# noisystreet/aither

Hardware: AMD Instinct MI355X
Metric: Mcell-updates/sec per iteration (residual+LU-SGS), 256^3 block; % HBM roofline (higher is better)
Workload: dtype f64

## Files before the change

### aither_amd/csrc/agx_api.hip

```cpp
#include "agx_kernels.hpp"
#include "agx_geometry.hpp"
#include "agx_mem.hpp"
#include <rccl/rccl.h>
#include <cstdarg>
#include <cstdio>
#include <cstring>
#include <cstdlib>
#include <cmath>
#include <vector>
#include <array>
#include <map>
#include <string>
#include <algorithm>

using namespace agx;

static char g_err[512] = "";
static int fail(const char* fmt, ...) {
  va_list ap;
  va_start(ap, fmt);
  vsnprintf(g_err, sizeof g_err, fmt, ap);
  va_end(ap);
  return 1;
}
// ... 1466 lines not shown
  if (cfg->equation_set != AGX_EQN_RANS || !cfg->is_viscous)
    return fail("the 7-equation library serves equation_set rans (viscous) only");
  if (cfg->turbulence_model != AGX_TURB_SST2003 && cfg->turbulence_model != AGX_TURB_KW_WILCOX2006 &&
      cfg->turbulence_model != AGX_TURB_SST_DES)
    return fail("turbulence_model %d: sst2003, sstdes and kOmegaWilcox2006 are built",
                cfg->turbulence_model);
  if (cfg->inv_flux_jacobian == AGX_JACOBIAN_APPROX_ROE)
    return fail("rans: approximateRoe is not built");
#else
  if (cfg->equation_set != AGX_EQN_EULER && cfg->equation_set != AGX_EQN_NAVIER_STOKES)
    return fail("equation_set %d: this library covers euler and navierStokes "
                "(rans: libaither_gfx950_rans.so)", cfg->equation_set);
  if ((cfg->equation_set == AGX_EQN_NAVIER_STOKES) != (cfg->is_viscous != 0))
    return fail("equation_set %d contradicts is_viscous %d", cfg->equation_set, cfg->is_viscous);
  if (cfg->turbulence_model != AGX_TURB_NONE)
    return fail("turbulence_model %d is not built (laminar / inviscid only)",
                cfg->turbulence_model);
#endif
  if (cfg->inv_flux_jacobian != AGX_JACOBIAN_RUSANOV &&
      cfg->inv_flux_jacobian != AGX_JACOBIAN_APPROX_ROE)
    return fail("inv_flux_jacobian %d is not one of rusanov / approximateRoe",
                cfg->inv_flux_jacobian);
  if (cfg->inv_flux_jacobian == AGX_JACOBIAN_APPROX_ROE && cfg->is_viscous)
    return fail("approximateRoe with viscous terms is not built: the reference hands dist and "
                "f1 to RoeOffDiagonal in swapped order (fluxJacobian.cpp:232 vs :240) and "
                "divides by f1 = 0 in laminar runs");
  if (cfg->viscous_recon != AGX_VISC_RECON_CENTRAL &&
      cfg->viscous_recon != AGX_VISC_RECON_CENTRAL_4TH)
    return fail("viscous_recon %d is not one of central / centralFourth", cfg->viscous_recon);
  if (cfg->viscous_recon == AGX_VISC_RECON_CENTRAL_4TH && cfg->n_ghost < 2)
    return fail("centralFourth needs two ghost layers (input::NumberGhostLayers, "
                "input.cpp:1127-1143)");
  if (cfg->matrix_solver < AGX_SOLVER_LUSGS || cfg->matrix_solver > AGX_SOLVER_BDPLUR)
    return fail("matrix_solver %d is not one of lusgs / dplur / blusgs / bdplur",
                cfg->matrix_solver);
  if ((cfg->matrix_solver == AGX_SOLVER_BLUSGS || cfg->matrix_solver == AGX_SOLVER_BDPLUR) &&
      cfg->inv_flux_jacobian == AGX_JACOBIAN_APPROX_ROE)
    return fail("block-matrix solvers are built for inviscidFluxJacobian rusanov only");
  c->cfg = *cfg;
  derive_gas(*cfg, c->gas);
  c->gas.wilcox = cfg->turbulence_model == AGX_TURB_KW_WILCOX2006 ? 1 : 0;
  c->gas.sstdes = cfg->turbulence_model == AGX_TURB_SST_DES ? 1 : 0;
  c->gas.turb_prandtl = c->gas.wilcox ? 8.0 / 9.0 : 0.9;
#if AGX_TPG
  c->gas.err = c->err_dev.get();
#endif
  SolverDev& sp = c->sp;
  sp.diag_add = 0;
  sp.kappa = cfg->kappa;
  sp.theta = cfg->theta;
  sp.zeta = cfg->zeta;
  sp.relax = cfg->matrix_relaxation;
  sp.dual_time_cfl = cfg->dual_time_cfl;
  sp.dt_fixed = cfg->dt_nondim;
  sp.visc_cfl_coeff = cfg->viscous_cfl_coeff;
  sp.viscous = cfg->is_viscous;
  sp.implicit = cfg->time_integration >= AGX_TIME_IMPLICIT_EULER;
  sp.bdf2 = cfg->time_integration == AGX_TIME_BDF2;
  sp.requires_init = cfg->matrix_solver == AGX_SOLVER_DPLUR ||
                     cfg->matrix_solver == AGX_SOLVER_BDPLUR || cfg->matrix_sweeps > 1;
  sp.block = (cfg->matrix_solver == AGX_SOLVER_BLUSGS || cfg->matrix_solver == AGX_SOLVER_BDPLUR) ? 1 : 0;
  sp.time_integration = cfg->time_integration;
  sp.roe_jacobian = cfg->inv_flux_jacobian == AGX_JACOBIAN_APPROX_ROE;
  c->have_cfg = true;
  return 0;
}

int agx_block_create(agx_ctx* c, const agx_block_geom* g, int* block_id) {
  if (!c->have_cfg) return fail("agx_config_set must precede agx_block_create");
  if (g->ng != c->cfg.n_ghost) return fail("block ghost layers != config n_ghost");
  if (g->ni < 1 || g->nj < 1 || g->nk < 1) return fail("empty block");
  const bool from_nodes = g->nodes != nullptr;
  if (from_nodes) {
    const double* arr[9] = {g->farea_i, g->farea_j, g->farea_k, g->vol, g->center, g->width_i,
                            g->width_j, g->width_k, g->wall_dist};
    const char* nm[9] = {"farea_i", "farea_j", "farea_k", "vol", "center", "width_i", "width_j",
                         "width_k", "wall_dist"};
    for (int q = 0; q < 9; ++q)
      if (arr[q])
        return fail("agx_block_create: nodes given together with %s (a block is built from "
                    "its nodes or from the nine arrays)", nm[q]);
  }
  if (!c->blocks.empty() && c->blocks[0].node_built != from_nodes)
    return fail("agx_block_create: a context holds node-built or array-built blocks, not both");
  HIPCHK(hipSetDevice(c->device));
  c->blocks.emplace_back();
  Block& b = c->blocks.back();
  BlockDev& d = b.d;
  memset(&d, 0, sizeof d);
  d.ni = g->ni; d.nj = g->nj; d.nk = g->nk; d.ng = g->ng;
  d.parent = g->parent_block;
  b.global_pos = g->global_pos;
  d.ioff = 16;
  const long row = d.ioff + d.ni + d.ng + 1;
  d.sx = (row + 15) / 16 * 16;
  d.sxy = d.sx * (d.nj + 2 * d.ng + 1);
  d.nplane = d.sxy * (d.nk + 2 * d.ng + 1);
  HIPCHK(b.slab.alloc((size_t)d.nplane * PL_COUNT));
  HIPCHK(hipMemsetAsync(b.slab.get(), 0, sizeof(double) * d.nplane * PL_COUNT, c->stream));
  auto pl = [&](int id) { return b.slab.get() + (long)id * d.nplane; };
  d.vol = pl(PL_VOL); d.specrad = pl(PL_SPECRAD); d.dt = pl(PL_DT);
  d.a = pl(PL_A); d.ainv = pl(PL_AINV); d.wdist = pl(PL_WDIST);
  for (int e = 0; e < AGX_NEQ; ++e) {
    d.state[e] = pl(PL_STATE_A + e); d.state2[e] = pl(PL_STATE_B + e);
    d.resid[e] = pl(PL_RESID + e); d.consn[e] = pl(PL_CONSN + e);
    d.consnm1[e] = pl(PL_CONSNM1 + e); d.x[e] = pl(PL_X + e);
    d.xold[e] = pl(PL_XOLD + e);
  }
  for (int q = 0; q < 3; ++q) {
    d.cen[q] = pl(PL_CEN + q);
    d.wid[q] = pl(PL_WID + q);
    for (int cc = 0; cc < 4; ++cc) d.fa[q][cc] = pl(PL_FA + 4 * q + cc);
  }
  b.state_is_a = true;
#if AGX_NEQ == 7
  d.specrad_t = pl(PL_SPECRAD_T); d.a_t = pl(PL_A_T); d.ainv_t = pl(PL_AINV_T);
  d.viscp = pl(PL_VISC);
  for (int q = 0; q < 3; ++q) d.turb3[q] = pl(PL_TURB3 + q);
#endif
  if (c->sp.implicit && is_block_solver(c)) {
    const size_t n = (size_t)d.nplane * (2 * AGX_NJ + 9 + 4);
    HIPCHK(b.blockmat.alloc(n));
    HIPCHK(hipMemsetAsync(b.blockmat.get(), 0, sizeof(double) * n, c->stream));
    d.am = b.blockmat.get();
    d.aminv = d.am + (size_t)d.nplane * AGX_NJ;
    d.vg = d.am + (size_t)d.nplane * 2 * AGX_NJ;
    d.am_t = d.vg + (size_t)d.nplane * 9;
    d.aminv_t = d.am_t + (size_t)d.nplane * 2;
  }
  d.sw_geo = d.sw_dyn = d.sw_rhs = nullptr;
  d.mg_forcing = d.mg_mres = d.mg_xsave = nullptr;
  if (c->sp.implicit && is_lusgs_solver(c) && !use_d2(c) && c->sweep_records) {
    const size_t n = (size_t)d.nplane * (SW_GEO + SW_DYN + SW_RHS);
    HIPCHK(b.sweep_rec.alloc(n));
    HIPCHK(hipMemsetAsync(b.sweep_rec.get(), 0, sizeof(double) * n, c->stream));
    d.sw_geo = b.sweep_rec.get();
    d.sw_dyn = d.sw_geo + (size_t)d.nplane * SW_GEO;
    d.sw_rhs = d.sw_dyn + (size_t)d.nplane * SW_DYN;
  }
  if (use_d2(c) && std::min(d.ni, d.nj) > KP_MAX_DIAG)
    return fail("LU-SGS: a block with min(ni, nj) = %d exceeds the %d cells per diagonal "
                "the sweep kernel holds in LDS (AGX_LUSGS=plane has no such limit)",
                std::min(d.ni, d.nj), KP_MAX_DIAG);
  if (use_d2(c)) {
    D2Dev& z = d.d2;
    z.Pi = d.ni + 2 * d.ng; z.Pj = d.nj + 2 * d.ng;
    z.ps = ((long)z.Pi * z.Pj + 15) / 16 * 16;
    z.nd2 = z.ps * (d.nk + 2 * d.ng);
    b.dstart.assign(z.Pi + z.Pj + 1, 0);
    std::vector<int> tab(z.Pi + z.Pj + 1 + (size_t)z.Pi * z.Pj);
    for (int de = 0; de < z.Pi + z.Pj - 1; ++de) {
      const int jl = std::max(0, de - (z.Pi - 1)), jh = std::min(z.Pj - 1, de);
      b.dstart[de + 1] = b.dstart[de] + (jh - jl + 1);
      for (int je = jl; je <= jh; ++je)
        tab[z.Pi + z.Pj + 1 + b.dstart[de] + (je - jl)] = (de - je) | (je << 16);
    }
    b.dstart[z.Pi + z.Pj] = b.dstart[z.Pi + z.Pj - 1];
    std::copy(b.dstart.begin(), b.dstart.end(), tab.begin());
    HIPCHK(b.d2_tab.upload(tab));
    z.dstart = b.d2_tab.get();
    z.ij_of_pos = z.dstart + z.Pi + z.Pj + 1;
    HIPCHK(b.d2.alloc((size_t)z.nd2 * D2_DOUBLES));
    HIPCHK(hipMemsetAsync(b.d2.get(), 0, sizeof(double) * z.nd2 * D2_DOUBLES, c->stream));
    z.base = b.d2.get();
  }
  b.node_built = from_nodes;
  if (from_nodes) {
    if (geo_block_metrics(c, b, g->nodes)) return 1;
    *block_id = (int)c->blocks.size() - 1;
    return 0;
  }
  const int ci = d.ni + 2 * d.ng, cj = d.nj + 2 * d.ng, ck = d.nk + 2 * d.ng;
  if (upload_aos(c, b, g->farea_i, d.fa[0], 4, ci + 1, cj, ck, d.ng)) return 1;
  if (upload_aos(c, b, g->farea_j, d.fa[1], 4, ci, cj + 1, ck, d.ng)) return 1;
  if (upload_aos(c, b, g->farea_k, d.fa[2], 4, ci, cj, ck + 1, d.ng)) return 1;
  double* volp[1] = {d.vol};
  if (upload_aos(c, b, g->vol, volp, 1, ci, cj, ck, d.ng)) return 1;
  if (upload_aos(c, b, g->center, d.cen, 3, ci, cj, ck, d.ng)) return 1;
  const double* wsrc[3] = {g->width_i, g->width_j, g->width_k};
  for (int q = 0; q < 3; ++q) {
    double* wp[1] = {d.wid[q]};
    if (upload_aos(c, b, wsrc[q], wp, 1, ci, cj, ck, d.ng)) return 1;
  }
#if AGX_FAST
  if (d.d2.base) {
    const long n = (long)d.d2.Pi * d.d2.Pj * (d.nk + 2 * d.ng);
    hipLaunchKernelGGL(k_d2_geo, dim3((n + 255) / 256), dim3(256), 0, c->stream, d);
  }
#endif
  HIPCHK(hipGetLastError());
  if (g->wall_dist) {
    double* wp[1] = {d.wdist};
    if (upload_aos(c, b, g->wall_dist, wp, 1, ci, cj, ck, d.ng)) return 1;
  }
  *block_id = (int)c->blocks.size() - 1;
  return 0;
}

int agx_block_set_bcs(agx_ctx* c, int id, int n, const agx_bc_surface* s) {
  if (id < 0 || id >= (int)c->blocks.size()) return fail("bad block id %d", id);
  Block& b = c->blocks[id];
  b.sweep_graph.drop();
  b.surf_host.assign(s, s + n);
  b.d.surf = nullptr;
  b.d.nsurf = 0;
  HIPCHK(b.surf_dev.alloc(n > 0 ? n : 1));
  HIPCHK(hipMemcpy(b.surf_dev.get(), s, sizeof(agx_bc_surface) * n, hipMemcpyHostToDevice));
  b.d.surf = b.surf_dev.get();
  b.d.nsurf = n;
  b.d.nsurf_i = b.d.nsurf_j = b.d.nsurf_k = 0;
  int n_conn[6] = {0, 0, 0, 0, 0, 0}, n_other[6] = {0, 0, 0, 0, 0, 0};
  for (int q = 0; q < n; ++q) {
    const int st = surface_type(s[q]);
    if (st <= 2) b.d.nsurf_i++; else if (st <= 4) b.d.nsurf_j++; else b.d.nsurf_k++;
    const int t = s[q].bc_type;
    if (t < AGX_BC_SLIPWALL || t > AGX_BC_PERIODIC) return fail("unknown bc type %d", t);
    if (t == AGX_BC_INTERBLOCK || t == AGX_BC_PERIODIC) n_conn[st - 1]++; else n_other[st - 1]++;
    if (t == AGX_BC_VISCOUSWALL && s[q].state.is_wall_law) {
      if (AGX_NEQ == 5) return fail("wallTreatment=wallLaw needs the rans library");
    }
  }
  for (int q = 0; q < 6; ++q)
    b.d.side_conn[q] = n_conn[q] == 0 ? 0 : (n_other[q] == 0 ? 1 : 2);
  b.d.nr_off = nullptr; b.d.nr_grad = nullptr; b.d.nr_mach = nullptr;
  b.nr_off_dev.reset();
  b.nr_mem.reset();
  b.nr_max = 0;
  std::vector<int> off(n > 0 ? n : 1, -1);
  long total = 0, nr_max = 0;
  for (int q = 0; q < n; ++q) {
    const int t = s[q].bc_type;
    if (!s[q].state.is_nonreflecting || (t != AGX_BC_INLET && t != AGX_BC_PRESSURE_OUTLET)) continue;
    const int st = surface_type(s[q]);
    const int d3 = (st - 1) / 2, d1 = (d3 + 1) % 3, d2 = (d3 + 2) % 3;
    const int lo[3] = {s[q].imin, s[q].jmin, s[q].kmin}, hi[3] = {s[q].imax, s[q].jmax, s[q].kmax};
    const long cells = (long)(hi[d1] - lo[d1]) * (hi[d2] - lo[d2]);
    off[q] = (int)total;
    total += cells;
    nr_max = std::max(nr_max, cells);
  }
  if (total > 0) {
    HIPCHK(b.nr_off_dev.upload(off.data(), (size_t)n));
    const size_t nd = (size_t)12 * total + 2 * (size_t)n;
    HIPCHK(b.nr_mem.alloc(nd));
    HIPCHK(hipMemset(b.nr_mem.get(), 0, sizeof(double) * nd));
    b.d.nr_off = b.nr_off_dev.get();
    b.d.nr_grad = b.nr_mem.get();
    b.d.nr_mach = b.nr_mem.get() + 12 * total;
    b.nr_max = nr_max;
  }
  b.d.wall_off = nullptr; b.d.wallv = nullptr;
  b.wall_off_dev.reset();
  b.wall_mem.reset();
  std::fill(off.begin(), off.end(), -1);
  total = 0;
  for (int q = 0; q < n; ++q) {
    if (s[q].bc_type != AGX_BC_VISCOUSWALL || !s[q].state.is_wall_law) continue;
    const int st = surface_type(s[q]);
    const int d3 = (st - 1) / 2, d1 = (d3 + 1) % 3, d2 = (d3 + 2) % 3;
    const int lo[3] = {s[q].imin, s[q].jmin, s[q].kmin}, hi[3] = {s[q].imax, s[q].jmax, s[q].kmax};
    off[q] = (int)total;
    total += (long)(hi[d1] - lo[d1]) * (hi[d2] - lo[d2]);
  }
  if (total > 0) {
    HIPCHK(b.wall_off_dev.upload(off.data(), (size_t)n));
    HIPCHK(b.wall_mem.alloc((size_t)total));
    HIPCHK(hipMemset(b.wall_mem.get(), 0, sizeof(WallVars) * (size_t)total));
    b.d.wall_off = b.wall_off_dev.get();
    b.d.wallv = b.wall_mem.get();
    c->have_wall_data = false;
  }
  b.wall_tab_dev.reset();
  b.wall_tab.clear();
  b.wall_faces = 0;
  for (int q = 0; q < n; ++q) {
    if (s[q].bc_type != AGX_BC_VISCOUSWALL) continue;
    WallSurfDev w;
    const int lo[3] = {s[q].imin, s[q].jmin, s[q].kmin}, hi[3] = {s[q].imax, s[q].jmax, s[q].kmax};
    const int nn[3] = {b.d.ni, b.d.nj, b.d.nk};
    w.side = surface_type(s[q]);
    const int d3 = (w.side - 1) / 2;
    for (int d = 0; d < 3; ++d) {
      w.lo[d] = lo[d];
      w.n[d] = d == d3 ? 1 : hi[d] - lo[d];
      if (lo[d] < 0 || hi[d] > nn[d] || w.n[d] < 1 || (d == d3 && lo[d] != 0 && lo[d] != nn[d]))
        return fail("viscousWall surface %d does not lie on a side of block %d", q, id);
    }
    w.off = b.wall_faces;
    b.wall_faces += (long)w.n[0] * w.n[1] * w.n[2];
    b.wall_tab.push_back(w);
  }
  HIPCHK(b.wall_tab_dev.upload(b.wall_tab));
  return 0;
}

int agx_conn_create(agx_ctx* c, const agx_connection* cc, int* conn_id) {
  c->conns.emplace_back();
  c->conns.back().c = *cc;
  *conn_id = (int)c->conns.size() - 1;
  return 0;
}

#ifndef AGX_MRESID_KC
#define AGX_MRESID_KC 32
#endif
constexpr int MRESID_KC = AGX_MRESID_KC;
long mresid_wgs(const agx_ctx* c, const BlockDev& b) {
  const long nchunk = ((long)b.d2.Pi * b.d2.Pj + 255) / 256;
  if (c->mresid_march) return 8L * ((nchunk + 7) / 8) * ((b.nk + MRESID_KC - 1) / MRESID_KC);
  const long bands = 8L * c->mresid_split;
  return bands * ((nchunk + bands - 1) / bands) * b.nk;
}

namespace {
int halo_batch_plan(agx_ctx* c, long* max_halo) {
  int sides = 0;
  long total = 0;
  std::vector<std::vector<unsigned char>> wlev(c->blocks.size()), rlev(c->blocks.size());
  auto flags = [&](std::vector<std::vector<unsigned char>>& v, int blk) -> std::vector<unsigned char>& {
    if (v[blk].empty()) v[blk].assign((size_t)c->blocks[blk].d.nplane, 0);
    return v[blk];
  };
  std::vector<std::pair<int, int>> order;
  int nlev = 0;
  for (size_t n = 0; n < c->conns.size(); ++n) {
    auto& k = c->conns[n];
    const agx_connection& cc = k.c;
    if (!(cc.rank[0] == c->rank && cc.rank[1] == c->rank)) continue;
    int lev = 1;
    for (int sd = 0; sd < 2; ++sd) {
      const auto& wr = flags(wlev, cc.local_block[1 - sd]);
      for (long q : k.side[sd].h_src) lev = std::max(lev, wr[(size_t)q] + 1);
      const auto& ww = flags(wlev, cc.local_block[sd]);
      const auto& rr = flags(rlev, cc.local_block[sd]);
      for (long q : k.side[sd].h_dst)
        lev = std::max(lev, std::max<int>(ww[(size_t)q] + 1, rr[(size_t)q]));
    }
    lev = std::min(lev, 250);
    for (int sd = 0; sd < 2; ++sd) {
      auto& rr = flags(rlev, cc.local_block[1 - sd]);
      for (long q : k.side[sd].h_src) rr[(size_t)q] = std::max<unsigned char>(rr[(size_t)q], lev);
      auto& ww = flags(wlev, cc.local_block[sd]);
      for (long q : k.side[sd].h_dst) ww[(size_t)q] = (unsigned char)lev;
      total += k.side[sd].n;
    }
    order.emplace_back(lev, (int)n);
    nlev = std::max(nlev, lev);
    sides += 2;
  }
  for (auto& k : c->conns)
    for (int sd = 0; sd < 2; ++sd) {
      std::vector<long>().swap(k.side[sd].h_dst);
      std::vector<long>().swap(k.side[sd].h_src);
    }
  c->halo_batch = c->halo_batch && sides >= 4 && nlev < 250 && 2 * nlev < sides;
  if (!c->halo_batch && c->halo_batch_required)
    return fail("AGX_HALO_BATCH=require: %d local connections in %d levels", sides / 2, nlev);
  if (!c->halo_batch) return 0;
  std::stable_sort(order.begin(), order.end(),
                   [](const std::pair<int, int>& x, const std::pair<int, int>& y) { return x.first < y.first; });
  c->halo_conn_order.clear();
  c->halo_levels.assign(nlev, agx_ctx::HaloLevel{0, 0, 0});
  long nmax_all = 0;
  for (auto& o : order) {
    auto& L = c->halo_levels[o.first - 1];
    if (L.sides == 0) L.first = 2 * (int)c->halo_conn_order.size();
    L.sides += 2;
    const auto& k = c->conns[o.second];
    L.nmax = std::max(L.nmax, std::max(k.side[0].n, k.side[1].n));
    nmax_all = std::max(nmax_all, L.nmax);
    c->halo_conn_order.push_back(o.second);
  }
  c->halo_batch_sides = sides;
  c->halo_batch_nmax = nmax_all;
  *max_halo = std::max(*max_halo, (total * AGX_NEQ + 1) / 2);
  HIPCHK(c->halo_tab_host.alloc((size_t)2 * sides));
  return 0;
}
void halo_sides(agx_ctx* c, Conn& k, int what, double* buf0, double* buf1, HaloSide* g,
                HaloSide* p) {
  Block& b0 = c->blocks[k.c.local_block[0]];
  Block& b1 = c->blocks[k.c.local_block[1]];
  const int z = halo_in_d2(b0, what);
  const auto &m0 = k.side[0].map[z], &m1 = k.side[1].map[z];
  g[0] = HaloSide{halo_planes(b1, what), m0.src.get(), k.side[0].n, buf0};
  g[1] = HaloSide{halo_planes(b0, what), m1.src.get(), k.side[1].n, buf1};
  p[0] = HaloSide{halo_planes(b0, what), m0.dst.get(), k.side[0].n, buf0};
  p[1] = HaloSide{halo_planes(b1, what), m1.dst.get(), k.side[1].n, buf1};
}
int halo_batch_tables(agx_ctx* c, int what) {
  const int set = c->halo_set[what];
  if (c->halo_tab_valid[what][set]) return 0;
  const int sides = c->halo_batch_sides;
  auto& tab = c->halo_tab_dev[what][set];
  for (int q = 0; q < 2; ++q)
    if (!tab[q]) HIPCHK(tab[q].alloc((size_t)sides));
  HIPCHK(hipStreamSynchronize(c->stream));
  HaloSide* g = c->halo_tab_host.get();
  HaloSide* p = g + sides;
  double* buf = c->halo_buf.get();
  int n = 0;
  for (int cid : c->halo_conn_order) {
    auto& k = c->conns[cid];
    const long n0 = k.side[0].n, n1 = k.side[1].n;
    halo_sides(c, k, what, buf, buf + n0 * AGX_NEQ, g + n, p + n);
    buf += (n0 + n1) * AGX_NEQ;
    n += 2;
  }
  HIPCHK(hipMemcpyAsync(tab[0].get(), g, sizeof(HaloSide) * sides, hipMemcpyHostToDevice,
                        c->stream));
  HIPCHK(hipMemcpyAsync(tab[1].get(), p, sizeof(HaloSide) * sides, hipMemcpyHostToDevice,
                        c->stream));
  c->halo_tab_valid[what][set] = true;
  return 0;
}
}

namespace {
struct CellIndex {
  const Block* b;
  int space;
  long operator()(int i, int j, int k) const {
    return !b ? 0L : space ? b->d2idx(i, j, k) : b->d.idx(i, j, k);
  }
};
int halo_maps(Conn& k, int s, int space, int ng, CellIndex idx_mine, CellIndex idx_partner,
              bool partner_local, long* max_halo) {
  MapOut m;
  build_side_map(k.c, s, ng, idx_mine, idx_partner, m);
  if (!partner_local) {
    MapOut ms;
    build_side_map(k.c, 1 - s, ng, idx_partner, idx_mine, ms);
    k.n_send = (long)ms.src.size();
    HIPCHK(k.send_src[space].upload(ms.src));
    *max_halo = std::max(*max_halo, (long)ms.src.size() * AGX_NEQ);
  }
  ConnSide& sd = k.side[s];
  sd.n = (long)m.dst.size();
  HIPCHK(sd.map[space].dst.upload(m.dst));
  if (partner_local) HIPCHK(sd.map[space].src.upload(m.src));
  *max_halo = std::max(*max_halo, (long)m.dst.size() * AGX_NEQ);
  if (space == 0) {
    sd.h_dst = std::move(m.dst);
    if (partner_local) sd.h_src = std::move(m.src);
  }
  return 0;
}
}

int agx_setup_finalize(agx_ctx* c) {
  HIPCHK(hipSetDevice(c->device));
  const int ng = c->cfg.n_ghost;
  if (!c->blocks.empty() && c->blocks[0].node_built && geo_complete(c)) return 1;
  long max_parts = 1, max_halo = 1;
  long march_parts = 0;
  for (auto& blk : c->blocks) {
    const dim3 g = cell_grid(blk.d, CELL_BLOCK);
    max_parts = std::max(max_parts, (long)g.x * g.y * g.z);
    march_parts += march_plan(c, blk.d).nparts;
    if (blk.d.d2.base)
      max_parts = std::max(max_parts, mresid_wgs(c, blk.d));
  }
  max_parts = std::max(max_parts, march_parts);
  for (auto& k : c->conns) {
    const agx_connection& cc = k.c;
    const bool l0 = cc.rank[0] == c->rank, l1 = cc.rank[1] == c->rank;
    if (!l0 && !l1) continue;
    for (int s = 0; s < 2; ++s) {
      const bool mine = s == 0 ? l0 : l1, partner_mine = s == 0 ? l1 : l0;
      if (!mine) continue;
      const int lb = cc.local_block[s];
      if (lb < 0 || lb >= (int)c->blocks.size()) return fail("connection refers to unknown block");
      const Block* partner = partner_mine ? &c->blocks[cc.local_block[1 - s]] : nullptr;
      for (int space = 0; space < (use_d2(c) ? 2 : 1); ++space)
        if (halo_maps(k, s, space, ng, CellIndex{&c->blocks[lb], space},
                      CellIndex{partner, space}, partner_mine, &max_halo))
          return 1;
    }
  }
  if (halo_batch_plan(c, &max_halo)) return 1;
  if (ensure_halo_buf(c, 2 * max_halo)) return 1;
  std::vector<std::pair<int, int>> per_peer;
  for (size_t n = 0; n < c->conns.size(); ++n) {
    if (my_side(c, c->conns[n]) < 0) continue;
    agx_ctx::Remote r;
    r.cid = (int)n;
    r.count = (long)agx_halo_count(c, (int)n, AGX_HALO_STATE);
    const bool hb = c->have_ex && c->ex.host_buffers;
    const size_t cap = (size_t)std::max<long>(r.count, 1);
    HIPCHK(r.send.alloc(cap));
    HIPCHK(r.recv.alloc(cap));
    if (hb) {
      HIPCHK(r.hsend.alloc(cap));
      HIPCHK(r.hrecv.alloc(cap));
    }
    const int s = my_side(c, c->conns[n]);
    agx_slab sl;
    sl.peer = c->conns[n].c.rank[1 - s];
    sl.tag = 0;
    bool seen = false;
    for (auto& pp : per_peer)
      if (pp.first == sl.peer) { sl.tag = pp.second++; seen = true; }
    if (!seen) per_peer.emplace_back(sl.peer, 1);
    sl.count = r.count;
    sl.send = hb ? r.hsend.get() : r.send.get();
    sl.recv = hb ? r.hrecv.get() : r.recv.get();
    c->slabs.push_back(sl);
    c->remote.push_back(std::move(r));
  }
  if (c->have_ex) {
    const size_t nrec = 1 + (size_t)c->ex.nranks;
    HIPCHK(c->rec_dev.alloc(nrec));
    HIPCHK(c->rec_host.alloc(nrec));
  }
  c->n_partials = max_parts;
  HIPCHK(c->partials.alloc((size_t)max_parts));
  const size_t nb = std::max<size_t>(c->blocks.size(), 1);
  HIPCHK(c->norm_out.alloc(2 * nb + 64));
  HIPCHK(c->norm_host.alloc(2 * nb));
  c->finalized = true;
  return 0;
}

int agx_state_upload(agx_ctx* c, int id, const double* state) {
  c->ghosts_prefilled = false;
  c->state_is_time_n = false;
  if (flush_consn(c)) return 1;
  if (id < 0 || id >= (int)c->blocks.size()) return fail("bad block id %d", id);
  Block& b = c->blocks[id];
  const BlockDev& d = b.d;
  if (upload_aos(c, b, state, d.state, AGX_NEQ, d.ni + 2 * d.ng,
                 d.nj + 2 * d.ng, d.nk + 2 * d.ng, d.ng))
    return 1;
#if AGX_NEQ == 7
  hipLaunchKernelGGL(k_aux_field, dim3((d.nplane + 255) / 256), dim3(256), 0, c->stream, d,
                     c->gas, 1, d.viscp);
  HIPCHK(hipGetLastError());
#endif
  return 0;
}

static int field_info(Block& b, int field, double* const** p, int* ncomp, int* ghost) {
  BlockDev& d = b.d;
  static thread_local double* one[1];
  switch (field) {
    case AGX_FIELD_STATE: *p = d.state; *ncomp = AGX_NEQ; *ghost = 1; return 0;
    case AGX_FIELD_RESIDUAL: *p = d.resid; *ncomp = AGX_NEQ; *ghost = 0; return 0;
    case AGX_FIELD_CONS_N: *p = d.consn; *ncomp = AGX_NEQ; *ghost = 0; return 0;
    case AGX_FIELD_CONS_NM1: *p = d.consnm1; *ncomp = AGX_NEQ; *ghost = 0; return 0;
    case AGX_FIELD_UPDATE: *p = d.x; *ncomp = AGX_NEQ; *ghost = 1; return 0;
    case AGX_FIELD_DT: one[0] = d.dt; *p = one; *ncomp = 1; *ghost = 0; return 0;
    case AGX_FIELD_SPEC_RADIUS: one[0] = d.specrad; *p = one; *ncomp = 1; *ghost = 0; return 0;
    case AGX_FIELD_DIAGONAL: one[0] = d.a; *p = one; *ncomp = 1; *ghost = 0; return 0;
  }
  return 1;
}
static int geom_field_info(Block& b, int field, double* const** p, int* ncomp, int* face) {
  BlockDev& d = b.d;
  static thread_local double* one[1];
  *face = -1;
  switch (field) {
    case AGX_FIELD_VOLUME: one[0] = d.vol; *p = one; *ncomp = 1; return 0;
    case AGX_FIELD_CENTER: *p = d.cen; *ncomp = 3; return 0;
    case AGX_FIELD_FAREA_I: case AGX_FIELD_FAREA_J: case AGX_FIELD_FAREA_K:
      *face = field - AGX_FIELD_FAREA_I; *p = d.fa[*face]; *ncomp = 4; return 0;
    case AGX_FIELD_WIDTH_I: case AGX_FIELD_WIDTH_J: case AGX_FIELD_WIDTH_K:
      one[0] = d.wid[field - AGX_FIELD_WIDTH_I]; *p = one; *ncomp = 1; return 0;
    case AGX_FIELD_WALL_DIST: one[0] = d.wdist; *p = one; *ncomp = 1; return 0;
  }
  return 1;
}

static int d2_x_copy(agx_ctx* c, Block& b, int to_d2) {
#if AGX_FAST
  b.x_planes_current = true;
  const long n = (long)b.d.d2.Pi * b.d.d2.Pj * (b.d.nk + 2 * b.d.ng);
  hipLaunchKernelGGL(k_d2_x_copy, dim3((n + 255) / 256), dim3(256), 0, c->stream, b.d, to_d2,
                     to_d2 ? (unsigned)(++b.kp_epoch) & 3u : 0u);
  HIPCHK(hipGetLastError());
#endif
  return 0;
}

static int ghosts_for_output(agx_ctx* c) {
  if (!c->ghosts_prefilled) {
    if (agx_phase_bc_faces(c)) return 1;
    if (agx_halo_swap_local(c, AGX_HALO_STATE)) return 1;
    if (agx_phase_bc_edges(c)) return 1;
  }
  if (c->cfg.is_viscous) {
    if (bc_pass(c, true, 2)) return 1;
    if (bc_pass(c, false, 1)) return 1;
  }
  c->ghosts_prefilled = false;
  return 0;
}

int agx_field_download(agx_ctx* c, int id, int field, double* out) {
  if (flush_consn(c)) return 1;
  if (id < 0 || id >= (int)c->blocks.size()) return fail("bad block id %d", id);
  Block& b = c->blocks[id];
  if (field == AGX_FIELD_UPDATE && b.d.d2.base && d2_x_copy(c, b, 0)) return 1;
  if (field >= AGX_FIELD_VEL_GRAD && field <= AGX_FIELD_PRESS_GRAD) {
    const long ncell = (long)b.d.ni * b.d.nj * b.d.nk;
    double* tmp = nullptr;
    if (ghosts_for_output(c)) return 1;
    if (stage_buffer(c, (size_t)3 * NGF * ncell, &tmp)) return 1;
// ... 1053 lines not shown
```

### aither_amd/csrc/agx_lusgs_kernels.hpp

```cpp
#pragma once

namespace agx {

constexpr int TT = 32;
constexpr int TRS = TT + 2;
__device__ __forceinline__ int tile_diag_index(int li, int lj) {
  const int dd = li + lj;
  if (dd < TT) return dd * (dd + 1) / 2 + lj;
  const int r = 2 * TT - 2 - dd;
  return TT * TT - (r + 1) * (r + 2) / 2 + (lj - (dd - (TT - 1)));
}
__device__ __forceinline__ void tile_table(unsigned short* s_tab) {
  const int tid = threadIdx.x;
#pragma unroll
  for (int m = 0; m < 4; ++m) {
    const int li = tid & (TT - 1), lj = (tid >> 5) + 8 * m;
    s_tab[tile_diag_index(li, lj)] = (unsigned short)(li | (lj << 8));
  }
}

__device__ __forceinline__ double kp_tagged(double v, unsigned tag) {
  const unsigned long long u = (unsigned long long)__double_as_longlong(v);
  return __longlong_as_double((long long)((u & ~3ull) | tag));
}
// ... 262 lines not shown
    const int kq = FWD ? k - 1 : k + 1;
    const bool has_pre = kt > 0;
    const bool k_any = has_pre || (CONN && b.side_conn[FWD ? 4 : 5] != 0);
    const long kbase = (long)(k + ng) * z.ps, qbase = (long)(kq + ng) * z.ps;
    auto step_geom = [&](int t, int& d, int& jmin, int& cnt, int& p0, int& pn) {
      d = FWD ? t : nsteps - 1 - t;
      jmin = max(0, d - (b.ni - 1));
      cnt = min(b.nj - 1, d) - jmin + 1;
      const int de = d + 2 * ng;
      p0 = z.dstart_cf(de) + (jmin + ng) - z.jlo(de);
      const int dq = FWD ? de - 1 : de + 1;
      pn = z.dstart_cf(dq) - z.jlo(dq);
    };
    auto fetch = [&](int t, KpCell* cc) {
      int d, jmin, cnt, p0, pn;
      step_geom(t, d, jmin, cnt, p0, pn);
#pragma unroll
      for (int m = 0; m < CH; ++m) {
        KpCell& c = cc[m];
        const int nraw = tid + 256 * m;
        c.act = nraw < cnt;
        const int n = c.act ? nraw : 0;
        c.j = jmin + n;
        c.i = d - c.j;
        c.pos = p0 + n;
        const unsigned vo = (unsigned)c.pos * 16u;
#pragma unroll
        for (int h = 0; h < 3; ++h) {
          c.o[h] = ld16(z.pab((FWD ? PA_B : PA_X) + h) + kbase * 16, vo);
          c.s[h] = ld16(z.pab(PA_S + h) + kbase * 16, vo);
          c.qs[h] = ld16(z.pab(PA_S + h) + qbase * 16, vo);
        }
        c.vf = ld8(z.vfb() + kbase * 8, (unsigned)c.pos * 8u);
        c.qvf = ld8(z.vfb() + qbase * 8, (unsigned)c.pos * 8u);
        const long fb[3] = {FWD ? kbase : kbase + pn, FWD ? kbase : kbase + pn + 1,
                            FWD ? kbase : kbase + z.ps};
        const unsigned fo[3] = {FWD ? vo : (unsigned)(c.j + ng) * 16u,
                                FWD ? vo : (unsigned)(c.j + ng) * 16u, vo};
#pragma unroll
        for (int q = 0; q < 3; ++q) {
          const double2 t0 = ld16(z.pab(PA_F + 2 * q) + fb[q] * 16, fo[q]);
          const double2 t1 = ld16(z.pab(PA_F + 2 * q + 1) + fb[q] * 16, fo[q]);
          c.f[q].n[0] = t0.x; c.f[q].n[1] = t0.y; c.f[q].n[2] = t1.x; c.f[q].a = t1.y;
          c.f[q].ad = ld8(z.adb(q) + fb[q] * 8, fo[q] >> 1);
        }
        const bool in_i = FWD ? c.i > 0 : c.i < b.ni - 1;
        const bool in_j = FWD ? c.j > 0 : c.j < b.nj - 1;
        int use = (in_i ? 1 : 0) | (in_j ? 2 : 0) | (has_pre ? 4 : 0);
        if (CONN) {
          if (FWD) {
            if (!in_i && bc_is_connection(b, c.i, c.j, k, 1)) use |= 1 | 8;
            if (!in_j && bc_is_connection(b, c.i, c.j, k, 3)) use |= 2 | 16;
            if (!has_pre && bc_is_connection(b, c.i, c.j, k, 5)) use |= 4;
          } else {
            if (!in_i && bc_is_connection(b, c.i + 1, c.j, k, 2)) use |= 1 | 8;
            if (!in_j && bc_is_connection(b, c.i, c.j + 1, k, 4)) use |= 2 | 16;
            if (!has_pre && bc_is_connection(b, c.i, c.j, k + 1, 6)) use |= 4;
          }
        }
        c.use = use;
      }
    };
    KpCell cur[CH], nxt[CH];
    double qx[CH][AGX_NEQ];
    auto qx_request = [&]() {
#pragma unroll
      for (int m = 0; m < CH; ++m) {
#pragma unroll
        for (int e = 0; e < AGX_NEQ; ++e) {
          const double* p = reinterpret_cast<const double*>(
              z.pab(PA_X + (e >> 1)) + qbase * 16 + (unsigned)cur[m].pos * 16u) + (e & 1);
          qx[m][e] = __hip_atomic_load(p, __ATOMIC_RELAXED, __HIP_MEMORY_SCOPE_AGENT);
        }
      }
    };
    auto qx_landed = [&]() {
      unsigned bad = 0;
#pragma unroll
      for (int m = 0; m < CH; ++m) {
#pragma unroll
        for (int e = 0; e < AGX_NEQ; ++e)
          bad |= cur[m].act ? ((unsigned)__double_as_longlong(qx[m][e]) ^ kp.tag) : 0u;
      }
      return (bad & 3u) == 0u;
    };
#pragma unroll
    for (int m = 0; m < CH; ++m) {
      cur[m].act = false;
#pragma unroll
      for (int e = 0; e < AGX_NEQ; ++e) qx[m][e] = 0.0;
    }
    int jmin_prev = 0;
    fetch(0, cur);
    __builtin_amdgcn_s_waitcnt(0x0F70);
    for (int t = 0; t < nsteps; ++t) {
      KP_STAMP(0);
      if (k_any) qx_request();
      fetch(min(t + 1, nsteps - 1), nxt);
      KP_STAMP(1);
      {
        int d, jmin, cnt, p0, pn;
      step_geom(t, d, jmin, cnt, p0, pn);
      double* lw = kp_lds + (size_t)(t & 1) * KP_NV * nsl;
      const double* lr = kp_lds + (size_t)((t & 1) ^ 1) * KP_NV * nsl;
      double accs[CH][AGX_NEQ];
#pragma unroll
      for (int m = 0; m < CH; ++m) {
        const KpCell& c = cur[m];
        double* acc = accs[m];
#pragma unroll
        for (int e = 0; e < AGX_NEQ; ++e) acc[e] = 0.0;
#pragma unroll
        for (int q = 0; q < 2; ++q) {
          const int jn = q == 0 ? c.j : (FWD ? c.j - 1 : c.j + 1);
          const double* rp = lr + min(max(jn - jmin_prev + 1, 0), nsl - 1);
          KpRec r;
#pragma unroll
          for (int e = 0; e < AGX_NEQ; ++e) r.dx[e] = rp[e * nsl];
          r.r1 = rp[5 * nsl]; r.v1[0] = rp[6 * nsl]; r.v1[1] = rp[7 * nsl]; r.v1[2] = rp[8 * nsl];
          r.p1 = rp[9 * nsl]; r.h1 = rp[10 * nsl];
          r.r0 = rp[11 * nsl]; r.v0[0] = rp[12 * nsl]; r.v0[1] = rp[13 * nsl]; r.v0[2] = rp[14 * nsl];
          r.p0 = rp[15 * nsl]; r.h0 = rp[16 * nsl]; r.cs = rp[17 * nsl]; r.vf = rp[18 * nsl];
          if (CONN && (c.use & (8 << q))) {
            const long pg = kbase + pn + (c.j + ng) + (q == 0 ? 0 : (FWD ? -1 : 1));
            kp_term_mem(z, g, visc, pg, c.f[q], FWD, acc);
          } else {
            const bool on = (c.use & (1 << q)) != 0;
            kp_term(r, c.f[q].n, on ? c.f[q].a : 0.0, on ? c.f[q].ad : 0.0, true, FWD, acc);
          }
        }
      }
      KP_STAMP(2);
      if (has_pre) {
        int spins = 0;
        while (!__all(qx_landed())) {
          __builtin_amdgcn_s_sleep(KP_SLEEP);
          if (++spins > kp.spin_limit ||
              ((spins & 63) == 0 &&
               __hip_atomic_load(kp.err, __ATOMIC_RELAXED, __HIP_MEMORY_SCOPE_AGENT) != 0)) {
            s_ok = 0;
            __hip_atomic_store(kp.err, 2, __ATOMIC_RELAXED, __HIP_MEMORY_SCOPE_AGENT);
            break;
          }
          qx_request();
          __builtin_amdgcn_s_waitcnt(0x0F70);
        }
      }
      KP_STAMP(3);
      __builtin_amdgcn_s_waitcnt(0x0F70);
#pragma unroll
      for (int m = 0; m < CH; ++m) {
        const KpCell& c = cur[m];
        double* acc = accs[m];
        const long own = kbase + c.pos;
        if (k_any) {
          const double qs5[AGX_NEQ] = {c.qs[0].x, c.qs[0].y, c.qs[1].x, c.qs[1].y, c.qs[2].x};
          KpRec r;
          kp_build_rec(g, qs5, c.qs[2].y, c.qvf, qx[m], r);
          const bool on = CONN ? (c.use & 4) != 0 : true;
          kp_term(r, c.f[2].n, on ? c.f[2].a : 0.0, on ? c.f[2].ad : 0.0, true, FWD, acc);
        }
        const double ainv = c.o[2].y;
        const double ov[AGX_NEQ] = {c.o[0].x, c.o[0].y, c.o[1].x, c.o[1].y, c.o[2].x};
        double xn[AGX_NEQ];
        if (FULL) {
          const int de = d + 2 * ng;
          const int dqo = FWD ? de + 1 : de - 1;
          const long po = kbase + z.dstart_cf(dqo) - z.jlo(dqo) + (c.j + ng);
          KpFace ff;
          if (FWD) {
            if (c.i < b.ni - 1 || bc_is_connection(b, c.i + 1, c.j, k, 2)) {
              kp_load_face(z, 0, po, visc, ff);
              kp_term_mem(z, g, visc, po, ff, false, acc);
            }
            if (c.j < b.nj - 1 || bc_is_connection(b, c.i, c.j + 1, k, 4)) {
              kp_load_face(z, 1, po + 1, visc, ff);
              kp_term_mem(z, g, visc, po + 1, ff, false, acc);
            }
            if (k < b.nk - 1 || bc_is_connection(b, c.i, c.j, k + 1, 6)) {
              kp_load_face(z, 2, own + z.ps, visc, ff);
              kp_term_mem(z, g, visc, own + z.ps, ff, false, acc);
            }
          } else {
            if (c.i > 0 || bc_is_connection(b, c.i, c.j, k, 1)) {
              kp_load_face(z, 0, own, visc, ff);
              kp_term_mem(z, g, visc, po, ff, true, acc);
            }
            if (c.j > 0 || bc_is_connection(b, c.i, c.j, k, 3)) {
              kp_load_face(z, 1, own, visc, ff);
              kp_term_mem(z, g, visc, po - 1, ff, true, acc);
            }
            if (k > 0 || bc_is_connection(b, c.i, c.j, k, 5)) {
              kp_load_face(z, 2, own, visc, ff);
              kp_term_mem(z, g, visc, own - z.ps, ff, true, acc);
            }
          }
          double bv[AGX_NEQ] = {ov[0], ov[1], ov[2], ov[3], ov[4]};
          if (!FWD) {
            const double2 b0 = z.ld_pair(PA_B, own), b1 = z.ld_pair(PA_B + 1, own),
                          b2 = z.ld_pair(PA_B + 2, own);
            bv[0] = b0.x; bv[1] = b0.y; bv[2] = b1.x; bv[3] = b1.y; bv[4] = b2.x;
          }
#pragma unroll
          for (int e = 0; e < AGX_NEQ; ++e) xn[e] = (bv[e] + acc[e]) * ainv;
        } else if (FWD) {
#pragma unroll
          for (int e = 0; e < AGX_NEQ; ++e) xn[e] = (ov[e] + acc[e]) * ainv;
        } else {
#pragma unroll
          for (int e = 0; e < AGX_NEQ; ++e) xn[e] = ov[e] + acc[e] * ainv;
        }
#pragma unroll
        for (int e = 0; e < AGX_NEQ; ++e) xn[e] = kp_tagged(xn[e], kp.tag);
        if (c.act) {
          typedef double v2d __attribute__((ext_vector_type(2)));
          const unsigned po = (unsigned)c.pos * 16u;
          const v2d v0 = {xn[0], xn[1]}, v1 = {xn[2], xn[3]}, v2 = {xn[4], ainv};
          asm volatile("s_nop 4\n\tglobal_store_dwordx4 %0, %1, %2 sc1\n\ts_nop 1"
                       :: "v"(po), "v"(v0), "s"(z.pab(PA_X + 0) + kbase * 16) : "memory");
          asm volatile("s_nop 4\n\tglobal_store_dwordx4 %0, %1, %2 sc1\n\ts_nop 1"
                       :: "v"(po), "v"(v1), "s"(z.pab(PA_X + 1) + kbase * 16) : "memory");
          asm volatile("s_nop 4\n\tglobal_store_dwordx4 %0, %1, %2 sc1\n\ts_nop 1"
                       :: "v"(po), "v"(v2), "s"(z.pab(PA_X + 2) + kbase * 16) : "memory");
        }
        const double s5[AGX_NEQ] = {c.s[0].x, c.s[0].y, c.s[1].x, c.s[1].y, c.s[2].x};
        KpRec r;
        kp_build_rec(g, s5, c.s[2].y, c.vf, xn, r);
        if (c.act) {
        double* wp = lw + (c.j - jmin + 1);
#pragma unroll
        for (int e = 0; e < AGX_NEQ; ++e) wp[e * nsl] = xn[e];
        wp[5 * nsl] = r.r1; wp[6 * nsl] = r.v1[0]; wp[7 * nsl] = r.v1[1]; wp[8 * nsl] = r.v1[2];
        wp[9 * nsl] = r.p1; wp[10 * nsl] = r.h1;
        wp[11 * nsl] = r.r0; wp[12 * nsl] = r.v0[0]; wp[13 * nsl] = r.v0[1]; wp[14 * nsl] = r.v0[2];
        wp[15 * nsl] = r.p0; wp[16 * nsl] = r.h0; wp[17 * nsl] = r.cs; wp[18 * nsl] = r.vf;
        }
      }
      jmin_prev = jmin;
      }
      KP_STAMP(4);
      __syncthreads();
      if (!s_ok) return;
#pragma unroll
      for (int m = 0; m < CH; ++m) cur[m] = nxt[m];
      KP_STAMP(5);
    }
  }
}

__global__ void __launch_bounds__(256)
k_matrix_resid_d2(BlockDev b, GasDev g, SolverDev sp, int nsplit, NormPartial* partials) {
  const D2Dev& z = b.d2;
  const int nchunk = (z.Pi * z.Pj + 255) / 256;
  const int per = (nchunk + 8 * nsplit - 1) / (8 * nsplit);
  const int xcd = blockIdx.x % 8, m = blockIdx.x / 8;
  const int band = (m / (per * b.nk)) * 8 + xcd, rem = m % (per * b.nk);
  const int k = rem / per, chunk = band * per + rem % per;
  const int t = chunk * 256 + threadIdx.x;
  const bool visc = sp.viscous != 0;
  double r[AGX_NEQ] = {0, 0, 0, 0, 0};
  bool active = false;
  if (chunk < nchunk && t < z.Pi * z.Pj) {
    const int ij = z.ij_of_pos[t];
    const int ie = ij & 0xffff, je = ij >> 16;
    const int i = ie - b.ng, j = je - b.ng;
    active = i >= 0 && i < b.ni && j >= 0 && j < b.nj;
    if (active) {
      const long kbase = (long)(k + b.ng) * z.ps;
      const long own = kbase + t;
      const int de = ie + je;
      const long plo = kbase + z.dstart[de - 1] - z.jlo(de - 1) + je;
      const long pup = kbase + z.dstart[de + 1] - z.jlo(de + 1) + je;
      double acc[AGX_NEQ] = {0, 0, 0, 0, 0};
      const long nlo[3] = {plo, plo - 1, own - z.ps}, nup[3] = {pup, pup + 1, own + z.ps};
      const int c3[3] = {i, j, k}, n3[3] = {b.ni, b.nj, b.nk};
      KpFace ff;
#pragma unroll
      for (int d = 0; d < 3; ++d) {
        if (c3[d] > 0 || bc_is_connection(b, i, j, k, 2 * d + 1)) {
          kp_load_face(z, d, own, visc, ff);
          kp_term_mem(z, g, visc, nlo[d], ff, true, acc);
        }
      }
#pragma unroll
      for (int d = 0; d < 3; ++d) {
        if (c3[d] < n3[d] - 1 ||
            bc_is_connection(b, i + (d == 0), j + (d == 1), k + (d == 2), 2 * d + 2)) {
          kp_load_face(z, d, nup[d], visc, ff);
          kp_term_mem(z, g, visc, nup[d], ff, false, acc);
        }
      }
      const double2 x0 = z.pa(PA_X)[own], x1 = z.pa(PA_X + 1)[own], x2 = z.pa(PA_X + 2)[own];
      const double2 b0 = z.pa(PA_B)[own], b1 = z.pa(PA_B + 1)[own], b2 = z.pa(PA_B + 2)[own];
      const double a = 1.0 / b2.y;
      const double xv[AGX_NEQ] = {x0.x, x0.y, x1.x, x1.y, x2.x};
      const double bv[AGX_NEQ] = {b0.x, b0.y, b1.x, b1.y, b2.x};
#pragma unroll
      for (int e = 0; e < AGX_NEQ; ++e) r[e] = -(xv[e] * a - acc[e] - bv[e]);
    }
  }
  norm_block_reduce(r, 0, active, partials + blockIdx.x);
}

#ifndef AGX_MR_WAVES
#define AGX_MR_WAVES 1
#endif
__global__ void __launch_bounds__(256, AGX_MR_WAVES)
k_matrix_resid_d2m(BlockDev b, GasDev g, SolverDev sp, int kc, NormPartial* partials) {
  const D2Dev& z = b.d2;
  const int nchunk = (z.Pi * z.Pj + 255) / 256;
  const int per = (nchunk + 7) / 8;
  const int xcd = blockIdx.x % 8, m = blockIdx.x / 8;
  const int chunk = xcd * per + m % per, kch = m / per;
  const int k0 = kch * kc, k1 = min(k0 + kc, b.nk);
  const int t = chunk * 256 + threadIdx.x;
  const bool visc = sp.viscous != 0;
  double l2[AGX_NEQ] = {0, 0, 0, 0, 0};
  bool active = false;
  int i = 0, j = 0, je = 0, de = 0;
  if (chunk < nchunk && t < z.Pi * z.Pj) {
    const int ij = z.ij_of_pos[t];
    const int ie = ij & 0xffff;
    je = ij >> 16;
    i = ie - b.ng; j = je - b.ng; de = ie + je;
    active = i >= 0 && i < b.ni && j >= 0 && j < b.nj;
  }
  if (active) {
    const long qlo = z.dstart[de - 1] - z.jlo(de - 1) + je;
    const long qup = z.dstart[de + 1] - z.jlo(de + 1) + je;
    struct Col { double s[AGX_NEQ], cs, x[AGX_NEQ], vf; };
    auto ld_col = [&](long p, Col& c) {
      const double2 s0 = z.ld_pair(PA_S, p), s1 = z.ld_pair(PA_S + 1, p), s2 = z.ld_pair(PA_S + 2, p);
      const double2 x0 = z.ld_pair(PA_X, p), x1 = z.ld_pair(PA_X + 1, p), x2 = z.ld_pair(PA_X + 2, p);
      c.s[0] = s0.x; c.s[1] = s0.y; c.s[2] = s1.x; c.s[3] = s1.y; c.s[4] = s2.x; c.cs = s2.y;
      c.x[0] = x0.x; c.x[1] = x0.y; c.x[2] = x1.x; c.x[3] = x1.y; c.x[4] = x2.x;
      c.vf = visc ? z.ld_vf(p) : 0.0;
    };
    auto col_term = [&](const Col& c, const KpFace& f, bool lower, double* acc) {
      KpRec r;
      kp_build_rec(g, c.s, c.cs, c.vf, c.x, r);
      kp_term(r, f.n, f.a, f.ad, visc, lower, acc);
    };
    Col cm, c0, cp;
    KpFace fk0, fk1;
    long own = (long)(k0 + b.ng) * z.ps + t;
    ld_col(own - z.ps, cm);
    ld_col(own, c0);
    kp_load_face(z, 2, own, visc, fk0);
    for (int k = k0; k < k1; ++k, own += z.ps) {
      const long kbase = own - t;
      ld_col(own + z.ps, cp);
      kp_load_face(z, 2, own + z.ps, visc, fk1);
      const double2 b0 = z.pa(PA_B)[own], b1 = z.pa(PA_B + 1)[own], b2 = z.pa(PA_B + 2)[own];
      double acc[AGX_NEQ] = {0, 0, 0, 0, 0};
      KpFace ff;
      if (i > 0 || bc_is_connection(b, i, j, k, 1)) {
        kp_load_face(z, 0, own, visc, ff);
        kp_term_mem(z, g, visc, kbase + qlo, ff, true, acc);
      }
      if (j > 0 || bc_is_connection(b, i, j, k, 3)) {
        kp_load_face(z, 1, own, visc, ff);
        kp_term_mem(z, g, visc, kbase + qlo - 1, ff, true, acc);
      }
      if (k > 0 || bc_is_connection(b, i, j, k, 5)) col_term(cm, fk0, true, acc);
      if (i < b.ni - 1 || bc_is_connection(b, i + 1, j, k, 2)) {
        kp_load_face(z, 0, kbase + qup, visc, ff);
        kp_term_mem(z, g, visc, kbase + qup, ff, false, acc);
      }
      if (j < b.nj - 1 || bc_is_connection(b, i, j + 1, k, 4)) {
        kp_load_face(z, 1, kbase + qup + 1, visc, ff);
        kp_term_mem(z, g, visc, kbase + qup + 1, ff, false, acc);
      }
      if (k < b.nk - 1 || bc_is_connection(b, i, j, k + 1, 6)) col_term(cp, fk1, false, acc);
      const double a = 1.0 / b2.y;
      const double bv[AGX_NEQ] = {b0.x, b0.y, b1.x, b1.y, b2.x};
#pragma unroll
      for (int e = 0; e < AGX_NEQ; ++e) {
        const double r = -(c0.x[e] * a - acc[e] - bv[e]);
        l2[e] += r * r;
      }
      cm = c0; c0 = cp; fk0 = fk1;
    }
  }
  norm_block_fold(l2, -1.0e300, 0x7fffffffffffffffLL, partials + blockIdx.x);
}

__global__ void __launch_bounds__(256)
k_update_d2(BlockDev b, GasDev g, SolverDev sp, int last_mm, NormPartial* partials) {
  __shared__ double sv[AGX_NEQ][TT][TRS];
  __shared__ unsigned short s_tab[TT * TT];
  const D2Dev& z = b.d2;
  const int tid = threadIdx.x;
  tile_table(s_tab);
  __syncthreads();
  const int i0 = blockIdx.x * TT, j0 = blockIdx.y * TT, k = blockIdx.z;
#pragma unroll
  for (int m = 0; m < 4; ++m) {
    const unsigned tl = s_tab[tid + 256 * m];
    const int tli = tl & 0xff, tlj = tl >> 8;
    const int i = i0 + tli, j = j0 + tlj;
    if (i < b.ni && j < b.nj) {
      const long p = (long)(k + b.ng) * z.ps + z.pos2(i + b.ng, j + b.ng);
      const double2 x0 = z.pa(PA_X)[p], x1 = z.pa(PA_X + 1)[p], x2 = z.pa(PA_X + 2)[p];
      sv[0][tlj][tli] = x0.x; sv[1][tlj][tli] = x0.y; sv[2][tlj][tli] = x1.x;
      sv[3][tlj][tli] = x1.y; sv[4][tlj][tli] = x2.x;
    }
  }
  __syncthreads();
  const int li = tid & (TT - 1);
  double l2[AGX_NEQ] = {0, 0, 0, 0, 0};
  double vmax = -1.0e300;
  long long vlin = 0x7fffffffffffffffLL;
#pragma unroll
  for (int m = 0; m < 4; ++m) {
    const int lj = (tid >> 5) + 8 * m;
    const int i = i0 + li, j = j0 + lj;
    if (i < b.ni && j < b.nj) {
      const long q = b.idx(i, j, k);
      double r[AGX_NEQ], s[AGX_NEQ], du[AGX_NEQ], ns[AGX_NEQ];
      load5(b.resid, q, r);
      load5(b.state, q, s);
#pragma unroll
      for (int e = 0; e < AGX_NEQ; ++e) du[e] = sv[e][lj][li];
      update_prim_with_cons(g, s, du, ns);
      store5(b.state, q, ns);
      if (sp.bdf2 && last_mm) {
        double u[AGX_NEQ];
        load5(b.consn, q, u);
        store5(b.consnm1, q, u);
      }
      const long lin0 = (((long)k * b.nj + j) * b.ni + i) * AGX_NEQ;
#pragma unroll
      for (int e = 0; e < AGX_NEQ; ++e) {
        l2[e] += r[e] * r[e];
        if (r[e] > vmax || (r[e] == vmax && lin0 + e < vlin)) { vmax = r[e]; vlin = lin0 + e; }
      }
    }
  }
  const long bid = ((long)blockIdx.z * gridDim.y + blockIdx.y) * gridDim.x + blockIdx.x;
  norm_block_fold(l2, vmax, vlin, partials + bid);
}

}
```

Measured before the change: 1477.

## Share i/j neighbor columns via wave shuffles in matrix residual kernel

Reworks the k-marching matrix-residual kernel so that the i-neighbor column is loaded once per plane and the j-neighbor column is obtained from the adjacent lane via __shfl_up/__shfl_down, falling back to a memory load only when that lane is inactive or out of range. The k-march now keeps two columns instead of three and reuses a single k-face load. The k chunk size is halved to expose more workgroups. These changes aim to cut redundant global loads of neighbor state, at the cost of extra shuffle instructions and possible register pressure, and they assume that adjacent lanes in the diagonal layout really hold the j-neighbors.

```diff
diff --git a/aither_amd/csrc/agx_api.hip b/aither_amd/csrc/agx_api.hip
--- a/aither_amd/csrc/agx_api.hip
+++ b/aither_amd/csrc/agx_api.hip
@@ -1792,7 +1792,7 @@
 }
 
 #ifndef AGX_MRESID_KC
-#define AGX_MRESID_KC 32
+#define AGX_MRESID_KC 16
 #endif
 constexpr int MRESID_KC = AGX_MRESID_KC;
 long mresid_wgs(const agx_ctx* c, const BlockDev& b) {
diff --git a/aither_amd/csrc/agx_lusgs_kernels.hpp b/aither_amd/csrc/agx_lusgs_kernels.hpp
--- a/aither_amd/csrc/agx_lusgs_kernels.hpp
+++ b/aither_amd/csrc/agx_lusgs_kernels.hpp
@@ -588,22 +588,18 @@
   norm_block_reduce(r, 0, active, partials + blockIdx.x);
 }
 
-#ifndef AGX_MR_WAVES
-#define AGX_MR_WAVES 1
-#endif
-__global__ void __launch_bounds__(256, AGX_MR_WAVES)
+__global__ void __launch_bounds__(256, 1)
 k_matrix_resid_d2m(BlockDev b, GasDev g, SolverDev sp, int kc, NormPartial* partials) {
   const D2Dev& z = b.d2;
+  const bool visc = sp.viscous != 0;
+  double l2[AGX_NEQ] = {0, 0, 0, 0, 0};
+  bool active = false;
+  int i = 0, j = 0, je = 0, de = 0, t = 0;
   const int nchunk = (z.Pi * z.Pj + 255) / 256;
   const int per = (nchunk + 7) / 8;
   const int xcd = blockIdx.x % 8, m = blockIdx.x / 8;
   const int chunk = xcd * per + m % per, kch = m / per;
-  const int k0 = kch * kc, k1 = min(k0 + kc, b.nk);
-  const int t = chunk * 256 + threadIdx.x;
-  const bool visc = sp.viscous != 0;
-  double l2[AGX_NEQ] = {0, 0, 0, 0, 0};
-  bool active = false;
-  int i = 0, j = 0, je = 0, de = 0;
+  t = chunk * 256 + threadIdx.x;
   if (chunk < nchunk && t < z.Pi * z.Pj) {
     const int ij = z.ij_of_pos[t];
     const int ie = ij & 0xffff;
@@ -611,6 +607,11 @@
     i = ie - b.ng; j = je - b.ng; de = ie + je;
     active = i >= 0 && i < b.ni && j >= 0 && j < b.nj;
   }
+  const int k0 = kch * kc, k1 = min(k0 + kc, b.nk);
+  const unsigned long long live = __ballot(active);
+  const int lane = threadIdx.x & 63;
+  const bool from_below = lane > 0 && ((live >> (lane - 1)) & 1) && je > z.jlo(de);
+  const bool from_above = lane < 63 && ((live >> (lane + 1)) & 1) && je < min(de, z.Pj - 1);
   if (active) {
     const long qlo = z.dstart[de - 1] - z.jlo(de - 1) + je;
     const long qup = z.dstart[de + 1] - z.jlo(de + 1) + je;
@@ -627,45 +628,70 @@
       kp_build_rec(g, c.s, c.cs, c.vf, c.x, r);
       kp_term(r, f.n, f.a, f.ad, visc, lower, acc);
     };
-    Col cm, c0, cp;
-    KpFace fk0, fk1;
+    auto col_of_lane = [&](const Col& c, int d, Col& o) {
+#pragma unroll
+      for (int e = 0; e < AGX_NEQ; ++e) {
+        o.s[e] = d < 0 ? __shfl_up(c.s[e], 1, 64) : __shfl_down(c.s[e], 1, 64);
+        o.x[e] = d < 0 ? __shfl_up(c.x[e], 1, 64) : __shfl_down(c.x[e], 1, 64);
+      }
+      o.cs = d < 0 ? __shfl_up(c.cs, 1, 64) : __shfl_down(c.cs, 1, 64);
+      o.vf = visc ? (d < 0 ? __shfl_up(c.vf, 1, 64) : __shfl_down(c.vf, 1, 64)) : 0.0;
+    };
+    auto plane_terms = [&](long own, int k, bool lower, double* acc) {
+      const long kbase = own - t;
+      KpFace ff;
+      Col ci, cj;
+      const long pn = kbase + (lower ? qlo : qup);
+      ld_col(pn, ci);
+      col_of_lane(ci, lower ? -1 : 1, cj);
+      if (!(lower ? from_below : from_above)) ld_col(lower ? pn - 1 : pn + 1, cj);
+      if (lower) {
+        if (i > 0 || bc_is_connection(b, i, j, k, 1)) {
+          kp_load_face(z, 0, own, visc, ff);
+          col_term(ci, ff, true, acc);
+        }
+        if (j > 0 || bc_is_connection(b, i, j, k, 3)) {
+          kp_load_face(z, 1, own, visc, ff);
+          col_term(cj, ff, true, acc);
+        }
+      } else {
+        if (i < b.ni - 1 || bc_is_connection(b, i + 1, j, k, 2)) {
+          kp_load_face(z, 0, pn, visc, ff);
+          col_term(ci, ff, false, acc);
+        }
+        if (j < b.nj - 1 || bc_is_connection(b, i, j + 1, k, 4)) {
+          kp_load_face(z, 1, pn + 1, visc, ff);
+          col_term(cj, ff, false, acc);
+        }
+      }
+    };
+    Col ca, cb;
+    KpFace fk;
+    double acc[AGX_NEQ] = {0, 0, 0, 0, 0}, bv[AGX_NEQ] = {0, 0, 0, 0, 0}, a = 1.0;
     long own = (long)(k0 + b.ng) * z.ps + t;
-    ld_col(own - z.ps, cm);
-    ld_col(own, c0);
-    kp_load_face(z, 2, own, visc, fk0);
-    for (int k = k0; k < k1; ++k, own += z.ps) {
-      const long kbase = own - t;
-      ld_col(own + z.ps, cp);
-      kp_load_face(z, 2, own + z.ps, visc, fk1);
-      const double2 b0 = z.pa(PA_B)[own], b1 = z.pa(PA_B + 1)[own], b2 = z.pa(PA_B + 2)[own];
-      double acc[AGX_NEQ] = {0, 0, 0, 0, 0};
-      KpFace ff;
-      if (i > 0 || bc_is_connection(b, i, j, k, 1)) {
-        kp_load_face(z, 0, own, visc, ff);
-        kp_term_mem(z, g, visc, kbase + qlo, ff, true, acc);
-      }
-      if (j > 0 || bc_is_connection(b, i, j, k, 3)) {
-        kp_load_face(z, 1, own, visc, ff);
-        kp_term_mem(z, g, visc, kbase + qlo - 1, ff, true, acc);
-      }
-      if (k > 0 || bc_is_connection(b, i, j, k, 5)) col_term(cm, fk0, true, acc);
-      if (i < b.ni - 1 || bc_is_connection(b, i + 1, j, k, 2)) {
-        kp_load_face(z, 0, kbase + qup, visc, ff);
-        kp_term_mem(z, g, visc, kbase + qup, ff, false, acc);
-      }
-      if (j < b.nj - 1 || bc_is_connection(b, i, j + 1, k, 4)) {
-        kp_load_face(z, 1, kbase + qup + 1, visc, ff);
-        kp_term_mem(z, g, visc, kbase + qup + 1, ff, false, acc);
-      }
-      if (k < b.nk - 1 || bc_is_connection(b, i, j, k + 1, 6)) col_term(cp, fk1, false, acc);
-      const double a = 1.0 / b2.y;
-      const double bv[AGX_NEQ] = {b0.x, b0.y, b1.x, b1.y, b2.x};
-#pragma unroll
-      for (int e = 0; e < AGX_NEQ; ++e) {
-        const double r = -(c0.x[e] * a - acc[e] - bv[e]);
-        l2[e] += r * r;
-      }
-      cm = c0; c0 = cp; fk0 = fk1;
+    ld_col(own - z.ps, ca);
+    for (int kk = k0; kk <= k1; ++kk, own += z.ps) {
+      ld_col(own, cb);
+      kp_load_face(z, 2, own, visc, fk);
+      if (kk > k0) {
+        if (kk < b.nk || bc_is_connection(b, i, j, kk, 6)) col_term(cb, fk, false, acc);
+#pragma unroll
+        for (int e = 0; e < AGX_NEQ; ++e) {
+          const double r = -(ca.x[e] * a - acc[e] - bv[e]);
+          l2[e] += r * r;
+        }
+      }
+      if (kk < k1) {
+        const double2 b0 = z.pa(PA_B)[own], b1 = z.pa(PA_B + 1)[own], b2 = z.pa(PA_B + 2)[own];
+#pragma unroll
+        for (int e = 0; e < AGX_NEQ; ++e) acc[e] = 0.0;
+        plane_terms(own, kk, true, acc);
+        if (kk > 0 || bc_is_connection(b, i, j, kk, 5)) col_term(ca, fk, true, acc);
+        plane_terms(own, kk, false, acc);
+        a = 1.0 / b2.y;
+        bv[0] = b0.x; bv[1] = b0.y; bv[2] = b1.x; bv[3] = b1.y; bv[4] = b2.x;
+      }
+      ca = cb;
     }
   }
   norm_block_fold(l2, -1.0e300, 0x7fffffffffffffffLL, partials + blockIdx.x);
```

Measured after the change: 1488 (median of 6 runs). Within noise of the previous version (+0.8%).
